# Byshx/Poccala

Hardware: AMD Instinct MI355X
Metric: frames/sec GMM-score+fwd-bwd, 39-d MFCC, 2048-mix (higher is better)
Workload: dtype f32-class (f16x2 split operands, f32 accumulate; f64 dynamic programming)

## Files before the change

### poccala_amd/csrc/gmm_accumulate_f16.hip

```cpp
#include <algorithm>

#include "pcl_internal.h"

namespace {

typedef float f16v __attribute__((ext_vector_type(16)));
typedef _Float16 h8v __attribute__((ext_vector_type(8)));
typedef _Float16 h4v __attribute__((ext_vector_type(4)));
typedef short s4v __attribute__((__vector_size__(4 * sizeof(short))));

#ifndef PCL_ACC16_AW
#define PCL_ACC16_AW 4
#endif
#ifndef PCL_ACC16_NSLOT
#define PCL_ACC16_NSLOT 6
#endif
constexpr int AW = PCL_ACC16_AW;
constexpr float FMAXH = 6.0e4f;
constexpr double LOG2E = 1.4426950408889634074;
constexpr float E_INIT = -1048576.f;
constexpr float G_TOP = 15.f;
constexpr float G_SET = 12.f;

__device__ __forceinline__ void glds16(const void *gsrc, unsigned int lds_dst) {
    unsigned int keep;
    lds_dst = __builtin_amdgcn_readfirstlane(lds_dst);
    asm volatile("s_mov_b32 %0, m0\n\ts_mov_b32 m0, %2\n\ts_nop 0\n\tglobal_load_lds_dwordx4 %1, off\n\ts_mov_b32 m0, %0"
                 : "=&s"(keep)
                 : "v"(gsrc), "s"(lds_dst)
                 : "memory");
}
__device__ __forceinline__ unsigned int lds_addr(const void *p) {
    return (unsigned int)(unsigned long long)(const __attribute__((address_space(3))) void *)p;
}

template <int D>
struct Img {
    static constexpr int KS = (D + 7) / 8;
    static constexpr int NCT = (KS + 1) / 2;
    static constexpr int B1 = 0;
    static constexpr int BM = 2 * KS;
    static constexpr int NB = BM + 1;
    static_assert(D % 8 != 0, "the folded constant needs a spare K slot");
};
__host__ __device__ constexpr int unit_of(int fg, int side, int s) { return (fg + side + 2 * (s & 1)) & 7; }

__global__ void acc16_tiles_kernel(const int *__restrict__ seg_lo, const int *__restrict__ seg_hi, const long long *__restrict__ off,
                                   int n_states, int *__restrict__ tile_off, int *__restrict__ state_flag) {
    __shared__ int part[1024];
    for (int w = threadIdx.x; w < n_states; w += blockDim.x) state_flag[w] = 0;
    const int tid = threadIdx.x, nt = blockDim.x;
    const int per = (n_states + nt - 1) / nt;
    const int lo = min(tid * per, n_states), hi = min(lo + per, n_states);
    int s = 0;
    for (int w = lo; w < hi; ++w) s += (int)((off[seg_hi[w]] - off[seg_lo[w]] + 31) / 32);
    part[tid] = s;
    __syncthreads();
    if (tid == 0) {
        int run = 0;
        for (int i = 0; i < nt; ++i) {
            const int v = part[i];
            part[i] = run;
            run += v;
        }
        tile_off[n_states] = run;
    }
    __syncthreads();
    int run = part[tid];
    for (int w = lo; w < hi; ++w) {
        tile_off[w] = run;
        run += (int)((off[seg_hi[w]] - off[seg_lo[w]] + 31) / 32);
    }
}

template <int D>
__global__ __launch_bounds__(256) void acc16_producer_kernel(
    const float *__restrict__ frames, const float *__restrict__ centers, const float *__restrict__ fscale,
    const double *__restrict__ kzero, int n_states, const int *__restrict__ work_states, const int *__restrict__ seg_lo,
    const int *__restrict__ seg_hi, const long long *__restrict__ off, const ActiveFrame *__restrict__ list, const int *__restrict__ tile_off, int tile_base,
    uint4 *__restrict__ images, unsigned int *__restrict__ tile_mask, int *__restrict__ state_flag) {
    using I = Img<D>;
    constexpr int KS = I::KS, XS = KS * 8 + 1;
    __shared__ float xs[32 * XS];
    __shared__ float cfs[32];
    __shared__ double lgs[32];
    __shared__ int s_state;
    __shared__ long long s_f0;
    __shared__ unsigned int s_mask;
    const int tid = threadIdx.x;
    const int n_tiles = tile_off[n_states];
    for (int tile = tile_base + blockIdx.x; tile < n_tiles; tile += gridDim.x) {
    __syncthreads();
    if (tid == 0) {
        int lo = 0, hi = n_states - 1;
        while (lo < hi) {
            const int mid = (lo + hi + 1) >> 1;
            if (tile_off[mid] <= tile) lo = mid; else hi = mid - 1;
        }
        s_state = lo;
        s_f0 = off[seg_lo[lo]] + 32LL * (tile - tile_off[lo]);
        s_mask = 0u;
    }
    __syncthreads();
    const int w = s_state, j = work_states[w];
    const long long f0 = s_f0;
    const int nf = (int)min(32LL, off[seg_hi[w]] - f0);
    const float *cen = centers + (size_t)j * D;
    for (int e = tid; e < 32 * KS * 8; e += 256) {
        const int f = e / (KS * 8), d = e - f * (KS * 8);
        float v = 0.f;
        if (f < nf && d < D) v = frames[list[f0 + f].frame * D + d] - cen[d];
        xs[f * XS + d] = v;
    }
    if (tid < 32) {
        double cf = -INFINITY, lg = 0.0;
        if (tid < nf) {
            const ActiveFrame a = list[f0 + tid];
            cf = a.coef * LOG2E + kzero[j];
            lg = a.lg;
        }
        cfs[tid] = (float)cf;
        lgs[tid] = lg;
    }
    __syncthreads();
    uint4 *img = images + (size_t)tile * (I::NB * 64);
    const float *fs = fscale + (size_t)j * 2 * (KS * 8);
    unsigned int ovf = 0u;
    for (int it = tid; it < KS * 64; it += 256) {
        const int s = it >> 6, ln = it & 63, side = ln >> 5, f = ln & 31;
        unsigned short h1[8], h2[8];
#pragma unroll
        for (int x = 0; x < 8; ++x) {
            const int d = 8 * s + x;
            float val = 0.f;
            if (d < D) {
                const float xc = xs[f * XS + d];
                val = (side ? xc : xc * xc) * fs[side * (KS * 8) + d];
                if (__builtin_fabsf(val) > FMAXH) ovf |= 1u << f;
                val = __builtin_fminf(__builtin_fmaxf(val, -FMAXH), FMAXH);
            } else if (d == D) {
                val = side ? 0.f : 1.f;
            }
            const _Float16 a = (_Float16)val;
            const _Float16 b = (d == D) ? (_Float16)0.f : (_Float16)(val - (float)a);
            h1[x] = __builtin_bit_cast(unsigned short, a);
            h2[x] = __builtin_bit_cast(unsigned short, b);
        }
        const int at = side * 32 + unit_of(f >> 2, side, s) * 4 + (f & 3);
        img[(I::B1 + 0 * KS + s) * 64 + at] = make_uint4(h1[0] | ((unsigned)h1[1] << 16), h1[2] | ((unsigned)h1[3] << 16), h1[4] | ((unsigned)h1[5] << 16), h1[6] | ((unsigned)h1[7] << 16));
        img[(I::B1 + 1 * KS + s) * 64 + at] = make_uint4(h2[0] | ((unsigned)h2[1] << 16), h2[2] | ((unsigned)h2[3] << 16), h2[4] | ((unsigned)h2[5] << 16), h2[6] | ((unsigned)h2[7] << 16));
    }
    if (ovf) atomicOr(&s_mask, ovf);
    __syncthreads();
    const unsigned int mask = s_mask;
    if (tid < 64) {
        unsigned int w4[4] = {0u, 0u, 0u, 0u};
        if (tid < 8) {
#pragma unroll
            for (int x = 0; x < 4; ++x) {
                const int q = tid * 4 + x, h = q >> 4, r = q & 15, f = (r & 3) + 8 * (r >> 2) + 4 * h;
                const float v = ((mask >> f) & 1u) ? -INFINITY : cfs[f];
                w4[x] = __float_as_uint(v);
            }
        } else if (tid >= 16 && tid < 32) {
            const int f = (tid - 16) * 2;
            const unsigned long long a = __double_as_longlong(lgs[f]), b = __double_as_longlong(lgs[f + 1]);
            w4[0] = (unsigned int)a; w4[1] = (unsigned int)(a >> 32);
            w4[2] = (unsigned int)b; w4[3] = (unsigned int)(b >> 32);
        }
        img[I::BM * 64 + tid] = make_uint4(w4[0], w4[1], w4[2], w4[3]);
    }
    if (tid == 0) {
        tile_mask[tile] = mask;
        if (mask) state_flag[w] = 1;
    }
    }
}

template <int D, bool FRESH>
__global__ __launch_bounds__(AW * 64, AW == 8 ? 1 : 2) void acc16_consumer_kernel(
    const uint4 *__restrict__ images, const uint4 *__restrict__ pm16f, const float *__restrict__ centers, const float *__restrict__ fscale,
    const double *__restrict__ means64, int M, int Mpad, int n_mtiles, int n_states, const int *__restrict__ work_states,
    const int *__restrict__ tile_off, int tile_base, double bias, double *__restrict__ st_acc, double *__restrict__ st_alpha,
    double *__restrict__ st_mean, double *__restrict__ st_cov, const int *__restrict__ npt, const int *__restrict__ nbad, const int *__restrict__ good_idx) {
    using I = Img<D>;
    constexpr int KS = I::KS, NCT = I::NCT, NB = I::NB;
    constexpr int NSLOT = PCL_ACC16_NSLOT;
    constexpr int AHEAD = NSLOT - 1;
    __shared__ __attribute__((aligned(16))) uint4 slot[NSLOT][NB * 64];

    const int nslice = (n_mtiles + AW - 1) / AW;
    const int b = blockIdx.x;
    const int w = (b & 7) + 8 * (b / (8 * nslice));
    const int slice = (b >> 3) % nslice;
    if (w >= n_states) return;
    const int t0 = tile_off[w] - tile_base, t1 = tile_off[w + 1] - tile_base;
    if (t0 == t1) return;
    const int j = work_states[w];
    const int lane = threadIdx.x & 63, half = lane >> 5, col = lane & 31;
    const int wave = __builtin_amdgcn_readfirstlane(threadIdx.x >> 6);
    const int mt = slice * AW + wave;
    const bool live = mt < npt[j];

    h8v pf[2][KS];
    {
        const uint4 *pq = pm16f + ((size_t)j * n_mtiles + (live ? mt : 0)) * (2 * KS * 64) + lane;
#pragma unroll
        for (int p = 0; p < 2; ++p)
#pragma unroll
            for (int s = 0; s < KS; ++s) pf[p][s] = __builtin_bit_cast(h8v, pq[(p * KS + s) * 64]);
    }
    f16v ST[NCT];
#pragma unroll
    for (int ct = 0; ct < NCT; ++ct)
#pragma unroll
        for (int r = 0; r < 16; ++r) ST[ct][r] = 0.f;
    float E = E_INIT;
    double galpha = 0.0;

    auto dma = [&](int t) {
        const uint4 *src = images + (size_t)t * (NB * 64);
        const unsigned int dst = __builtin_amdgcn_readfirstlane(lds_addr(&slot[t % NSLOT][0]));
#pragma unroll
        for (int k = 0; k < (NB + AW - 1) / AW; ++k) {
            const int p = wave + k * AW;
            if (p < NB) glds16(src + p * 64 + lane, dst + (unsigned int)p * 1024u);
        }
    };
    const int row_even = half * 32 + unit_of(col >> 2, half, 0) * 4 + (col & 3);
    const int row_odd = half * 32 + unit_of(col >> 2, half, 1) * 4 + (col & 3);
    auto load1 = [&](int t, uint4 (&a1)[KS], uint4 (&a2)[KS]) {
        const uint4 *x1 = &slot[t % NSLOT][I::B1 * 64];
#pragma unroll
        for (int s = 0; s < KS; ++s) a2[s] = x1[(1 * KS + s) * 64 + ((s & 1) ? row_odd : row_even)];
#pragma unroll
        for (int s = 0; s < KS; ++s) a1[s] = x1[(0 * KS + s) * 64 + ((s & 1) ? row_odd : row_even)];
    };
    auto mfma1 = [&](const uint4 (&a1)[KS], const uint4 (&a2)[KS], f16v &d) {
#pragma unroll
        for (int s = 0; s < KS; ++s) d = __builtin_amdgcn_mfma_f32_32x32x16_f16(__builtin_bit_cast(h8v, a2[s]), pf[0][s], d, 0, 0, 0);
#pragma unroll
        for (int s = 0; s < KS; ++s) d = __builtin_amdgcn_mfma_f32_32x32x16_f16(__builtin_bit_cast(h8v, a1[s]), pf[1][s], d, 0, 0, 0);
#pragma unroll
        for (int s = 0; s < KS; ++s) d = __builtin_amdgcn_mfma_f32_32x32x16_f16(__builtin_bit_cast(h8v, a1[s]), pf[0][s], d, 0, 0, 0);
    };
    const int tg = (lane >> 4) & 1, tq = (lane >> 2) & 3, tp = lane & 3;
    int tr_off[4];
#pragma unroll
    for (int k = 0; k < 4; ++k)
        tr_off[k] = tg * 1024 + (tp >> 1) * 512 + unit_of(2 * k + half, tp >> 1, tg) * 64 + tq * 16 + 8 * (tp & 1);
    auto load2 = [&](int t, int sp, uint4 (&x)[2][NCT]) {
        const unsigned char *base = reinterpret_cast<const unsigned char *>(&slot[t % NSLOT][I::B1 * 64]);
#pragma unroll
        for (int p = 0; p < 2; ++p)
#pragma unroll
            for (int ct = 0; ct < NCT; ++ct) {
                const s4v lo = __builtin_amdgcn_ds_read_tr16_b64_v4i16((__attribute__((address_space(3))) s4v *)(base + tr_off[2 * sp] + p * KS * 1024 + ct * 2048));
                const s4v hi = __builtin_amdgcn_ds_read_tr16_b64_v4i16((__attribute__((address_space(3))) s4v *)(base + tr_off[2 * sp + 1] + p * KS * 1024 + ct * 2048));
                const uint2 l2 = __builtin_bit_cast(uint2, lo), h2 = __builtin_bit_cast(uint2, hi);
                x[p][ct] = make_uint4(l2.x, l2.y, h2.x, h2.y);
            }
    };
    auto mfma2 = [&](const uint4 &g1, const uint4 &g2, const uint4 (&x)[2][NCT]) {
#pragma unroll
        for (int ct = 0; ct < NCT; ++ct) ST[ct] = __builtin_amdgcn_mfma_f32_32x32x16_f16(__builtin_bit_cast(h8v, x[1][ct]), __builtin_bit_cast(h8v, g1), ST[ct], 0, 0, 0);
#pragma unroll
        for (int ct = 0; ct < NCT; ++ct) ST[ct] = __builtin_amdgcn_mfma_f32_32x32x16_f16(__builtin_bit_cast(h8v, x[0][ct]), __builtin_bit_cast(h8v, g2), ST[ct], 0, 0, 0);
#pragma unroll
        for (int ct = 0; ct < NCT; ++ct) ST[ct] = __builtin_amdgcn_mfma_f32_32x32x16_f16(__builtin_bit_cast(h8v, x[0][ct]), __builtin_bit_cast(h8v, g1), ST[ct], 0, 0, 0);
    };

    constexpr int MYB_HI = (NB + AW - 1) / AW, MYB_LO = NB / AW;
    const bool more_blocks = wave < NB % AW;
    for (int k = 0; k < AHEAD; ++k)
        if (t0 + k < t1) dma(t0 + k);
    __builtin_amdgcn_s_waitcnt(0x0F70);
    __syncthreads();
    f16v dA, dB;
#pragma unroll
    for (int r = 0; r < 16; ++r) dA[r] = dB[r] = 0.f;
    uint4 a1[KS], a2[KS];
    auto load_cf = [&](int t, f16v &c) {
        const float4 *cfp = reinterpret_cast<const float4 *>(&slot[t % NSLOT][I::BM * 64]) + half * 4;
#pragma unroll
        for (int q = 0; q < 4; ++q) {
            const float4 v = cfp[q];
            c[4 * q] = v.x; c[4 * q + 1] = v.y; c[4 * q + 2] = v.z; c[4 * q + 3] = v.w;
        }
    };
    auto tile_max = [&](const f16v &d) -> float {
        float m3 = __builtin_fmaxf(__builtin_fmaxf(d[0], d[1]), d[2]);
#pragma unroll
        for (int r = 3; r < 15; r += 2) m3 = __builtin_fmaxf(__builtin_fmaxf(m3, d[r]), d[r + 1]);
        m3 = __builtin_fmaxf(m3, d[15]);
        const auto sw = __builtin_amdgcn_permlane32_swap(__float_as_uint(m3), __float_as_uint(m3), false, false);
        return __builtin_fmaxf(__uint_as_float(sw[0]), __uint_as_float(sw[1]));
    };
    float mx = -INFINITY;
    if (live) {
        load1(t0, a1, a2);
        load_cf(t0, dA);
        mfma1(a1, a2, dA);
        load_cf(t0 + 1, dB);
        load1(t0 + 1, a1, a2);
        mx = tile_max(dA);
    }
    auto tile_step = [&](int t, f16v &d1, f16v &dn) __attribute__((always_inline)) {
        const bool ahead = t + AHEAD < t1;
        if (ahead) dma(t + AHEAD);
        const uint4 *cur = &slot[t % NSLOT][0];
        if (slice == 0 && wave == 0 && lane < 32) galpha += reinterpret_cast<const double *>(cur + I::BM * 64)[32 + lane];
        if (live) {
            const float rel = mx - E;
            if (__builtin_amdgcn_ballot_w64(rel > G_TOP) != 0ull) {
                const float delta = rel > G_TOP ? __builtin_ceilf(rel) - G_SET : 0.f;
                const float f = __builtin_amdgcn_exp2f(-delta);
                E += delta;
#pragma unroll
                for (int ct = 0; ct < NCT; ++ct)
#pragma unroll
                    for (int r = 0; r < 16; ++r) ST[ct][r] *= f;
            }
            uint4 x0[2][NCT], x1[2][NCT];
            unsigned int u1[8], u2[8];
#pragma unroll
            for (int r = 0; r < 8; ++r) {
                const float ga = __builtin_amdgcn_exp2f(d1[2 * r] - E), gb = __builtin_amdgcn_exp2f(d1[2 * r + 1] - E);
                u1[r] = __builtin_bit_cast(unsigned int, __builtin_amdgcn_cvt_pkrtz(ga, gb));
                const float ra = ga - (float)__builtin_bit_cast(_Float16, (unsigned short)(u1[r] & 0xffffu));
                const float rb = gb - (float)__builtin_bit_cast(_Float16, (unsigned short)(u1[r] >> 16));
                u2[r] = __builtin_bit_cast(unsigned int, __builtin_amdgcn_cvt_pkrtz(ra, rb));
            }
            const uint4 g1a = make_uint4(u1[0], u1[1], u1[2], u1[3]), g1b = make_uint4(u1[4], u1[5], u1[6], u1[7]);
            const uint4 g2a = make_uint4(u2[0], u2[1], u2[2], u2[3]), g2b = make_uint4(u2[4], u2[5], u2[6], u2[7]);
            mfma1(a1, a2, dn);
            load2(t, 0, x0);
            load2(t, 1, x1);
            mfma2(g1a, g2a, x0);
            mfma2(g1b, g2b, x1);
            load_cf(t + 2, d1);
            load1(t + 2, a1, a2);
            mx = tile_max(dn);
#ifndef PCL_ACC16_NOSGB
            {
                constexpr int RX = 8 * NCT, RY = 4 + 2 * KS, NY = 6 * NCT, PERX = (RX + 2) / 3, PERY = (RY + NY - 1) / NY;
#pragma unroll
                for (int i = 0; i < 3; ++i) {
                    __builtin_amdgcn_sched_group_barrier(0x008, KS, 0);
                    __builtin_amdgcn_sched_group_barrier(0x100, PERX, 0);
                }
#pragma unroll
                for (int i = 0; i < NY; ++i) {
                    __builtin_amdgcn_sched_group_barrier(0x008, 1, 0);
                    __builtin_amdgcn_sched_group_barrier(0x100, PERY, 0);
                }
            }
#endif
        }
        static_assert(MYB_HI * (AHEAD - 3) <= 16 && AHEAD >= 3, "counted waits below");
        {
            const int newest = min(t + AHEAD, t1 - 1);
            const int keep = max(0, newest - (t + 3)) * (more_blocks ? MYB_HI : MYB_LO);
            switch (keep) {
#define W(N) case N: asm volatile("s_waitcnt vmcnt(" #N ")" ::: "memory"); break;
                W(0) W(1) W(2) W(3) W(4) W(5) W(6) W(7) W(8) W(9) W(10) W(11) W(12) W(13) W(14) W(15)
#undef W
                default: asm volatile("s_waitcnt vmcnt(16)" ::: "memory"); break;
            }
        }
        __builtin_amdgcn_s_barrier();
    };
    for (int t = t0; t < t1; t += 2) {
        tile_step(t, dA, dB);
        if (t + 1 < t1) tile_step(t + 1, dB, dA);
    }

    if (!live) return;
    const int row_ = mt * 32 + col, nb_ = nbad[j];
    const int m = good_idx ? ((row_ < M - nb_) ? (nb_ ? good_idx[(size_t)j * Mpad + row_] : row_) : M) : row_;
    constexpr int C0 = ((KS - 1) & 1) * 16 + (D & 7), CT0 = (KS - 1) >> 1;
    constexpr int R0 = (C0 & 3) + 4 * (C0 >> 3), H0 = (C0 >> 2) & 1;
    float s0f = ST[CT0][R0];
    {
        const auto sw = __builtin_amdgcn_permlane32_swap(__float_as_uint(s0f), __float_as_uint(s0f), false, false);
        s0f = __uint_as_float(H0 ? sw[1] : sw[0]);
    }
    const int Ei = (int)E;
    const double S0 = ldexp((double)s0f, Ei);
    if (m < M) {
        const float *cen = centers + (size_t)j * D;
        const float *fs = fscale + (size_t)j * 2 * (KS * 8);
#pragma unroll
        for (int ct = 0; ct < NCT; ++ct)
#pragma unroll
            for (int r = 0; r < 16; ++r) {
                if (r & 4) continue;
                const int c = (r & 3) + 8 * (r >> 2) + 4 * half, s = 2 * ct + (c >> 4), d = 8 * s + (c & 7);
                if (s >= KS || d >= D) continue;
                const size_t o = ((size_t)j * Mpad + m) * D + d;
                const double cc = (double)cen[d], dl = means64[o] - cc;
                const double S2 = ldexp((double)ST[ct][r], Ei) / (double)fs[d], S1 = ldexp((double)ST[ct][r + 4], Ei) / (double)fs[KS * 8 + d];
                const double vm = S1 + (cc + bias) * S0;
                const double vc = fmax(S2 - 2.0 * dl * S1 + dl * dl * S0, 0.0);
                if (FRESH) {
                    st_mean[o] = vm;
                    st_cov[o] = vc;
                } else {
                    st_mean[o] += vm;
                    st_cov[o] += vc;
                }
            }
        if (half == 0) {
            if (FRESH) st_acc[(size_t)j * Mpad + m] = S0;
            else st_acc[(size_t)j * Mpad + m] += S0;
        }
    }
    if (slice == 0 && wave == 0) {
        double v = (lane < 32) ? galpha : 0.0;
#pragma unroll
        for (int o = 32; o > 0; o >>= 1) v += __shfl_xor(v, o, 64);
        if (lane == 0) st_alpha[j] += v;
    }
}

}

size_t pcl_acc16_image_bytes(int D) {
    switch (D) {
#define CASE(DD) case DD: return (size_t)Img<DD>::NB * 1024;
        PCL_MFMA_DIMS(CASE)
#undef CASE
        default: return 0;
    }
}

int pcl_launch_acc16_produce(pcl_ctx *ctx, int first, int ns, int max_tiles, int buf, hipStream_t stream) {
    if (ns == 0) return PCL_OK;
    AccScratch &a = ctx->acc;
    const int *ws = a.work_states.p + first, *lo = a.seg_lo.p + first, *hi = a.seg_hi.p + first;
    hipLaunchKernelGGL(acc16_tiles_kernel, dim3(1), dim3(1024), 0, stream, lo, hi, a.off.p, ns, a.tile_off[buf].p, a.state_flag[buf].p);
    const int pgrid = std::max(1, std::min(max_tiles, std::max(ctx->cus, 1) * 16));
    switch (ctx->D) {
#define PRODUCE16(DD)                                                                                                                              \
    case DD: hipLaunchKernelGGL((acc16_producer_kernel<DD>), dim3(pgrid), dim3(256), 0, stream, ctx->frames32, ctx->centers32, ctx->fscale,        \
                                ctx->kzero, ns, ws, lo, hi, a.off.p, a.list.p, a.tile_off[buf].p, 0, reinterpret_cast<uint4 *>(a.images[buf].p),   \
                                a.tile_mask[buf].p, a.state_flag[buf].p); break;
        PCL_MFMA_DIMS(PRODUCE16)
#undef PRODUCE16
        default: PCL_FAIL(ctx, PCL_ERR_INVALID, "internal: no f16 accumulate kernel for D=%d", ctx->D);
    }
    HIPCHK(ctx, hipGetLastError());
    return PCL_OK;
}

int pcl_launch_acc16_consume(pcl_ctx *ctx, int first, int ns, int buf, bool fresh, hipStream_t stream) {
    if (ns == 0) return PCL_OK;
    AccScratch &a = ctx->acc;
    const int nmt = ctx->Mpad32 / 32, nslice = (nmt + AW - 1) / AW;
    const int nblocks = ((ns + 7) / 8) * 8 * nslice;
    const int *ws = a.work_states.p + first;
#define CONSUME16F(DD, FR)                                                                                                    \
    hipLaunchKernelGGL((acc16_consumer_kernel<DD, FR>), dim3(nblocks), dim3(AW * 64), 0, stream,                              \
                       reinterpret_cast<const uint4 *>(a.images[buf].p), reinterpret_cast<const uint4 *>(ctx->pm16f.p), ctx->centers32, ctx->fscale, \
                       ctx->mean64, ctx->M, ctx->Mpad, nmt, ns, ws, a.tile_off[buf].p, 0, 100.0, ctx->st_acc, ctx->st_alpha,      \
                       ctx->st_mean, ctx->st_cov, ctx->d_npt, ctx->d_nbad, (ctx->compact_main && ctx->D <= 48) ? ctx->d_good_idx : (const int *)nullptr)
    switch (ctx->D) {
#define CONSUME16(DD) case DD: if (fresh) CONSUME16F(DD, true); else CONSUME16F(DD, false); break;
        PCL_MFMA_DIMS(CONSUME16)
#undef CONSUME16
        default: PCL_FAIL(ctx, PCL_ERR_INVALID, "internal: no f16 accumulate kernel for D=%d", ctx->D);
    }
#undef CONSUME16F
    HIPCHK(ctx, hipGetLastError());
    return PCL_OK;
}
```

Measured before the change: 21.17 million.

## Pack odd K-slice tail into shared MFMA tile to drop half-empty column tile

Splits the second-product accumulators into full column tiles plus a tail, and rotates the layout of the last hi/lo slice so the tail's split-precision cross terms share one MFMA. This cuts the per-step MFMA count for odd KS (D=39) by avoiding a half-wasted 32x32 tile. It adds an extra accumulator register block and more complex epilogue summation, which may raise register pressure.

```diff
diff --git a/poccala_amd/csrc/gmm_accumulate_f16.hip b/poccala_amd/csrc/gmm_accumulate_f16.hip
--- a/poccala_amd/csrc/gmm_accumulate_f16.hip
+++ b/poccala_amd/csrc/gmm_accumulate_f16.hip
@@ -37,13 +37,16 @@
 template <int D>
 struct Img {
     static constexpr int KS = (D + 7) / 8;
-    static constexpr int NCT = (KS + 1) / 2;
+    static constexpr int NFT = KS / 2;
+    static constexpr bool TAIL = (KS & 1) != 0;
     static constexpr int B1 = 0;
     static constexpr int BM = 2 * KS;
     static constexpr int NB = BM + 1;
     static_assert(D % 8 != 0, "the folded constant needs a spare K slot");
+    static_assert(NFT >= 1, "product (2) is laid out for at least one full row tile");
+    static constexpr int rot(int p, int s) { return (s & 1) ^ (int)(TAIL && p == 1 && s == KS - 1); }
 };
-__host__ __device__ constexpr int unit_of(int fg, int side, int s) { return (fg + side + 2 * (s & 1)) & 7; }
+__host__ __device__ constexpr int unit_of(int fg, int side, int rot) { return (fg + side + 2 * (rot & 1)) & 7; }
 
 __global__ void acc16_tiles_kernel(const int *__restrict__ seg_lo, const int *__restrict__ seg_hi, const long long *__restrict__ off,
                                    int n_states, int *__restrict__ tile_off, int *__restrict__ state_flag) {
@@ -146,9 +149,10 @@
             h1[x] = __builtin_bit_cast(unsigned short, a);
             h2[x] = __builtin_bit_cast(unsigned short, b);
         }
-        const int at = side * 32 + unit_of(f >> 2, side, s) * 4 + (f & 3);
-        img[(I::B1 + 0 * KS + s) * 64 + at] = make_uint4(h1[0] | ((unsigned)h1[1] << 16), h1[2] | ((unsigned)h1[3] << 16), h1[4] | ((unsigned)h1[5] << 16), h1[6] | ((unsigned)h1[7] << 16));
-        img[(I::B1 + 1 * KS + s) * 64 + at] = make_uint4(h2[0] | ((unsigned)h2[1] << 16), h2[2] | ((unsigned)h2[3] << 16), h2[4] | ((unsigned)h2[5] << 16), h2[6] | ((unsigned)h2[7] << 16));
+        const int at1 = side * 32 + unit_of(f >> 2, side, I::rot(0, s)) * 4 + (f & 3);
+        const int at2 = side * 32 + unit_of(f >> 2, side, I::rot(1, s)) * 4 + (f & 3);
+        img[(I::B1 + 0 * KS + s) * 64 + at1] = make_uint4(h1[0] | ((unsigned)h1[1] << 16), h1[2] | ((unsigned)h1[3] << 16), h1[4] | ((unsigned)h1[5] << 16), h1[6] | ((unsigned)h1[7] << 16));
+        img[(I::B1 + 1 * KS + s) * 64 + at2] = make_uint4(h2[0] | ((unsigned)h2[1] << 16), h2[2] | ((unsigned)h2[3] << 16), h2[4] | ((unsigned)h2[5] << 16), h2[6] | ((unsigned)h2[7] << 16));
     }
     if (ovf) atomicOr(&s_mask, ovf);
     __syncthreads();
@@ -184,7 +188,8 @@
     const int *__restrict__ tile_off, int tile_base, double bias, double *__restrict__ st_acc, double *__restrict__ st_alpha,
     double *__restrict__ st_mean, double *__restrict__ st_cov, const int *__restrict__ npt, const int *__restrict__ nbad, const int *__restrict__ good_idx) {
     using I = Img<D>;
-    constexpr int KS = I::KS, NCT = I::NCT, NB = I::NB;
+    constexpr int KS = I::KS, NFT = I::NFT, NB = I::NB;
+    constexpr bool TAIL = I::TAIL;
     constexpr int NSLOT = PCL_ACC16_NSLOT;
     constexpr int AHEAD = NSLOT - 1;
     __shared__ __attribute__((aligned(16))) uint4 slot[NSLOT][NB * 64];
@@ -210,11 +215,14 @@
 #pragma unroll
             for (int s = 0; s < KS; ++s) pf[p][s] = __builtin_bit_cast(h8v, pq[(p * KS + s) * 64]);
     }
-    f16v ST[NCT];
-#pragma unroll
-    for (int ct = 0; ct < NCT; ++ct)
-#pragma unroll
-        for (int r = 0; r < 16; ++r) ST[ct][r] = 0.f;
+    f16v ST[NFT];
+    f16v STt, STu;
+#pragma unroll
+    for (int r = 0; r < 16; ++r) {
+#pragma unroll
+        for (int ct = 0; ct < NFT; ++ct) ST[ct][r] = 0.f;
+        STt[r] = STu[r] = 0.f;
+    }
     float E = E_INIT;
     double galpha = 0.0;
 
@@ -232,9 +240,9 @@
     auto load1 = [&](int t, uint4 (&a1)[KS], uint4 (&a2)[KS]) {
         const uint4 *x1 = &slot[t % NSLOT][I::B1 * 64];
 #pragma unroll
-        for (int s = 0; s < KS; ++s) a2[s] = x1[(1 * KS + s) * 64 + ((s & 1) ? row_odd : row_even)];
-#pragma unroll
-        for (int s = 0; s < KS; ++s) a1[s] = x1[(0 * KS + s) * 64 + ((s & 1) ? row_odd : row_even)];
+        for (int s = 0; s < KS; ++s) a2[s] = x1[(1 * KS + s) * 64 + (I::rot(1, s) ? row_odd : row_even)];
+#pragma unroll
+        for (int s = 0; s < KS; ++s) a1[s] = x1[(0 * KS + s) * 64 + (I::rot(0, s) ? row_odd : row_even)];
     };
     auto mfma1 = [&](const uint4 (&a1)[KS], const uint4 (&a2)[KS], f16v &d) {
 #pragma unroll
@@ -249,25 +257,34 @@
 #pragma unroll
     for (int k = 0; k < 4; ++k)
         tr_off[k] = tg * 1024 + (tp >> 1) * 512 + unit_of(2 * k + half, tp >> 1, tg) * 64 + tq * 16 + 8 * (tp & 1);
-    auto load2 = [&](int t, int sp, uint4 (&x)[2][NCT]) {
+    const int tail_off = (tg + 1) * (KS - 1) * 1024;
+    auto load2 = [&](int t, int sp, uint4 (&x)[2][NFT], uint4 &xt) {
         const unsigned char *base = reinterpret_cast<const unsigned char *>(&slot[t % NSLOT][I::B1 * 64]);
+        if (TAIL) {
+            const s4v lo = __builtin_amdgcn_ds_read_tr16_b64_v4i16((__attribute__((address_space(3))) s4v *)(base + tr_off[2 * sp] + tail_off));
+            const s4v hi = __builtin_amdgcn_ds_read_tr16_b64_v4i16((__attribute__((address_space(3))) s4v *)(base + tr_off[2 * sp + 1] + tail_off));
+            const uint2 l2 = __builtin_bit_cast(uint2, lo), h2 = __builtin_bit_cast(uint2, hi);
+            xt = make_uint4(l2.x, l2.y, h2.x, h2.y);
+        }
 #pragma unroll
         for (int p = 0; p < 2; ++p)
 #pragma unroll
-            for (int ct = 0; ct < NCT; ++ct) {
+            for (int ct = 0; ct < NFT; ++ct) {
                 const s4v lo = __builtin_amdgcn_ds_read_tr16_b64_v4i16((__attribute__((address_space(3))) s4v *)(base + tr_off[2 * sp] + p * KS * 1024 + ct * 2048));
                 const s4v hi = __builtin_amdgcn_ds_read_tr16_b64_v4i16((__attribute__((address_space(3))) s4v *)(base + tr_off[2 * sp + 1] + p * KS * 1024 + ct * 2048));
                 const uint2 l2 = __builtin_bit_cast(uint2, lo), h2 = __builtin_bit_cast(uint2, hi);
                 x[p][ct] = make_uint4(l2.x, l2.y, h2.x, h2.y);
             }
     };
-    auto mfma2 = [&](const uint4 &g1, const uint4 &g2, const uint4 (&x)[2][NCT]) {
-#pragma unroll
-        for (int ct = 0; ct < NCT; ++ct) ST[ct] = __builtin_amdgcn_mfma_f32_32x32x16_f16(__builtin_bit_cast(h8v, x[1][ct]), __builtin_bit_cast(h8v, g1), ST[ct], 0, 0, 0);
-#pragma unroll
-        for (int ct = 0; ct < NCT; ++ct) ST[ct] = __builtin_amdgcn_mfma_f32_32x32x16_f16(__builtin_bit_cast(h8v, x[0][ct]), __builtin_bit_cast(h8v, g2), ST[ct], 0, 0, 0);
-#pragma unroll
-        for (int ct = 0; ct < NCT; ++ct) ST[ct] = __builtin_amdgcn_mfma_f32_32x32x16_f16(__builtin_bit_cast(h8v, x[0][ct]), __builtin_bit_cast(h8v, g1), ST[ct], 0, 0, 0);
+    auto mfma2 = [&](const uint4 &g1, const uint4 &g2, const uint4 (&x)[2][NFT], const uint4 &xt) {
+        if (TAIL) STu = __builtin_amdgcn_mfma_f32_32x32x16_f16(__builtin_bit_cast(h8v, xt), __builtin_bit_cast(h8v, g2), STu, 0, 0, 0);
+#pragma unroll
+        for (int ct = 0; ct < NFT; ++ct) ST[ct] = __builtin_amdgcn_mfma_f32_32x32x16_f16(__builtin_bit_cast(h8v, x[1][ct]), __builtin_bit_cast(h8v, g1), ST[ct], 0, 0, 0);
+#pragma unroll
+        for (int ct = 0; ct < NFT; ++ct) ST[ct] = __builtin_amdgcn_mfma_f32_32x32x16_f16(__builtin_bit_cast(h8v, x[0][ct]), __builtin_bit_cast(h8v, g2), ST[ct], 0, 0, 0);
+        if (TAIL) STt = __builtin_amdgcn_mfma_f32_32x32x16_f16(__builtin_bit_cast(h8v, xt), __builtin_bit_cast(h8v, g1), STt, 0, 0, 0);
+#pragma unroll
+        for (int ct = 0; ct < NFT; ++ct) ST[ct] = __builtin_amdgcn_mfma_f32_32x32x16_f16(__builtin_bit_cast(h8v, x[0][ct]), __builtin_bit_cast(h8v, g1), ST[ct], 0, 0, 0);
     };
 
     constexpr int MYB_HI = (NB + AW - 1) / AW, MYB_LO = NB / AW;
@@ -317,11 +334,18 @@
                 const float f = __builtin_amdgcn_exp2f(-delta);
                 E += delta;
 #pragma unroll
-                for (int ct = 0; ct < NCT; ++ct)
+                for (int ct = 0; ct < NFT; ++ct)
 #pragma unroll
                     for (int r = 0; r < 16; ++r) ST[ct][r] *= f;
-            }
-            uint4 x0[2][NCT], x1[2][NCT];
+                if (TAIL) {
+#pragma unroll
+                    for (int r = 0; r < 16; ++r) {
+                        STt[r] *= f;
+                        STu[r] *= f;
+                    }
+                }
+            }
+            uint4 x0[2][NFT], x1[2][NFT], xt0 = {}, xt1 = {};
             unsigned int u1[8], u2[8];
 #pragma unroll
             for (int r = 0; r < 8; ++r) {
@@ -334,16 +358,16 @@
             const uint4 g1a = make_uint4(u1[0], u1[1], u1[2], u1[3]), g1b = make_uint4(u1[4], u1[5], u1[6], u1[7]);
             const uint4 g2a = make_uint4(u2[0], u2[1], u2[2], u2[3]), g2b = make_uint4(u2[4], u2[5], u2[6], u2[7]);
             mfma1(a1, a2, dn);
-            load2(t, 0, x0);
-            load2(t, 1, x1);
-            mfma2(g1a, g2a, x0);
-            mfma2(g1b, g2b, x1);
+            load2(t, 0, x0, xt0);
+            load2(t, 1, x1, xt1);
+            mfma2(g1a, g2a, x0, xt0);
+            mfma2(g1b, g2b, x1, xt1);
             load_cf(t + 2, d1);
             load1(t + 2, a1, a2);
             mx = tile_max(dn);
 #ifndef PCL_ACC16_NOSGB
             {
-                constexpr int RX = 8 * NCT, RY = 4 + 2 * KS, NY = 6 * NCT, PERX = (RX + 2) / 3, PERY = (RY + NY - 1) / NY;
+                constexpr int RX = 8 * NFT + (TAIL ? 4 : 0), RY = 4 + 2 * KS, NY = 6 * NFT + (TAIL ? 4 : 0), PERX = (RX + 2) / 3, PERY = (RY + NY - 1) / NY;
 #pragma unroll
                 for (int i = 0; i < 3; ++i) {
                     __builtin_amdgcn_sched_group_barrier(0x008, KS, 0);
@@ -380,26 +404,37 @@
     const int m = good_idx ? ((row_ < M - nb_) ? (nb_ ? good_idx[(size_t)j * Mpad + row_] : row_) : M) : row_;
     constexpr int C0 = ((KS - 1) & 1) * 16 + (D & 7), CT0 = (KS - 1) >> 1;
     constexpr int R0 = (C0 & 3) + 4 * (C0 >> 3), H0 = (C0 >> 2) & 1;
-    float s0f = ST[CT0][R0];
-    {
-        const auto sw = __builtin_amdgcn_permlane32_swap(__float_as_uint(s0f), __float_as_uint(s0f), false, false);
-        s0f = __uint_as_float(H0 ? sw[1] : sw[0]);
-    }
+    auto from_half = [&](float v) -> double {
+        const auto sw = __builtin_amdgcn_permlane32_swap(__float_as_uint(v), __float_as_uint(v), false, false);
+        return (double)__uint_as_float(H0 ? sw[1] : sw[0]);
+    };
     const int Ei = (int)E;
-    const double S0 = ldexp((double)s0f, Ei);
+    double s0;
+    if constexpr (TAIL) s0 = from_half(STt[R0]) + from_half(STt[R0 + 8]) + from_half(STu[R0]);
+    else s0 = from_half(ST[CT0 < NFT ? CT0 : 0][R0]);
+    const double S0 = ldexp(s0, Ei);
     if (m < M) {
         const float *cen = centers + (size_t)j * D;
         const float *fs = fscale + (size_t)j * 2 * (KS * 8);
 #pragma unroll
-        for (int ct = 0; ct < NCT; ++ct)
+        for (int ct = 0; ct < NFT + (TAIL ? 1 : 0); ++ct)
 #pragma unroll
             for (int r = 0; r < 16; ++r) {
                 if (r & 4) continue;
+                if (ct == NFT && r >= 8) continue;
                 const int c = (r & 3) + 8 * (r >> 2) + 4 * half, s = 2 * ct + (c >> 4), d = 8 * s + (c & 7);
-                if (s >= KS || d >= D) continue;
+                if (d >= D) continue;
                 const size_t o = ((size_t)j * Mpad + m) * D + d;
                 const double cc = (double)cen[d], dl = means64[o] - cc;
-                const double S2 = ldexp((double)ST[ct][r], Ei) / (double)fs[d], S1 = ldexp((double)ST[ct][r + 4], Ei) / (double)fs[KS * 8 + d];
+                double s2, s1;
+                if (ct < NFT) {
+                    s2 = (double)ST[ct < NFT ? ct : 0][r];
+                    s1 = (double)ST[ct < NFT ? ct : 0][r + 4];
+                } else {
+                    s2 = (double)STt[r & 7] + (double)STt[(r & 7) + 8] + (double)STu[r & 7];
+                    s1 = (double)STt[(r & 7) + 4] + (double)STt[(r & 7) + 12] + (double)STu[(r & 7) + 4];
+                }
+                const double S2 = ldexp(s2, Ei) / (double)fs[d], S1 = ldexp(s1, Ei) / (double)fs[KS * 8 + d];
                 const double vm = S1 + (cc + bias) * S0;
                 const double vc = fmax(S2 - 2.0 * dl * S1 + dl * dl * S0, 0.0);
                 if (FRESH) {
```

Result: no change. 21.17 million, median of 2 (-0.0%).
